# rezasalatin/PINN_depthEstimation

Measured on AMD Instinct MI355X. Metric: collocation-point residuals/sec (fwd+PDE-grad+Adam), higher is better.
Workload: dtype f32; 1 GPU; BASELINE configs[1]: 3->8x64 tanh->4 MLP, Navier_Stokes residual, 1048576 synthetic (t,x,y) points per GPU, full-batch Adam step; points_per_gpu=1048576, global_points=1048576, params=29636, parallelism=dp1, engine=0, allreduce_bytes=0

## Files before the change

pinn_depthestimation_amd/csrc/fused_kernel.h:

```cpp
#pragma once
#include <string.h>
#include <type_traits>
#include "common.h"
#include "residuals.h"

namespace pinn {

typedef float f4 __attribute__((ext_vector_type(4)));

constexpr int FUSED_WAVES = 4;
constexpr int FUSED_W16_WAVES = 3;
constexpr int FUSED_FLUSH_ROWS = 4;
constexpr int FUSED_THREADS = FUSED_WAVES * 64;
constexpr int TB_FLOATS = 256;
constexpr int TB_PER_WAVE = 8;
constexpr int MAX_SUMS = 12;
constexpr int MSE_SUM0 = 4;

struct FusedParams {
  int d_in, d_out, L, act;
  int dir_col[PINN_MAX_DIRS];
  int64_t N, n_tiles;
  const float* X;
  const float* Wp;
  const float* WTp;
  const float* Bp;
  float* scratch;
  int64_t scratch_per_wave;
  float* Y; float* dY;
  int loss_kind;
  int residual_id;
  int out_col[PINN_MAX_ROLES];
  int q_of[PINN_MAX_DIRS];
  float thr, anchor; int xcol;
  const float* scale;
  int n_cols;
  int mse_col[PINN_MAX_ROLES];
  const float* T;
  int64_t n_split;
  const float* mse_scale;
  float* wg_sums;
  float* wg_grads;
  int acc_lds;
  int PW, PB;
  int lds_acc_floats;
  int batch_T;
  int io1;
  uint32_t drop_seed, drop_thresh;
  float drop_scale, drop_keep;
  const float* gY;
  const float* gdY;
};

__device__ __forceinline__ f4 mfma4(float a, float b, f4 c) {
  return __builtin_amdgcn_mfma_f32_16x16x4f32(a, b, c, 0, 0, 0);
}

template <int WP> __device__ __forceinline__ int w_off_p(int l) { return l == 0 ? 0 : WP * 16 + (l - 1) * WP * WP; }
template <int WP> __device__ __forceinline__ int b_off_p(int l) { return l * WP; }

template <int NT_IN, int NT_OUT>
__device__ __forceinline__ void load_w(const float* __restrict__ Wl, f4 (&w)[NT_OUT][NT_IN], int m, int kq) {
  constexpr int LDW = 16 * NT_IN;
#pragma unroll
  for (int MT = 0; MT < NT_OUT; ++MT)
#pragma unroll
    for (int kt = 0; kt < NT_IN; ++kt)
      w[MT][kt] = *reinterpret_cast<const f4*>(Wl + (16 * MT + m) * LDW + 16 * kt + 4 * kq);
}

template <int NT_IN, int NT_OUT, int K1, int KR = 4>
__device__ __forceinline__ void gemm_chain(const f4 (&w)[NT_OUT][NT_IN], const f4 (&bin)[K1][NT_IN],
                                           f4 (&acc)[K1][NT_OUT]) {
#pragma unroll
  for (int MT = 0; MT < NT_OUT; ++MT)
#pragma unroll
    for (int kt = 0; kt < NT_IN; ++kt)
#pragma unroll
      for (int r = 0; r < KR; ++r)
#pragma unroll
        for (int c = 0; c < K1; ++c) acc[c][MT] = mfma4(w[MT][kt][r], bin[c][kt][r], acc[c][MT]);
}


template <int NT_IN>
__device__ __forceinline__ void load_wblk(const float* __restrict__ Wl, int MT, f4 (&w)[NT_IN], int m, int kq) {
#pragma unroll
  for (int kt = 0; kt < NT_IN; ++kt)
    w[kt] = *reinterpret_cast<const f4*>(Wl + (16 * MT + m) * (16 * NT_IN) + 16 * kt + 4 * kq);
}

struct NoMid { __device__ __forceinline__ void operator()() const {} };
template <int NT_IN, int NT_OUT, int K1, class Mid = NoMid>
__device__ __forceinline__ void gemm_stream(const float* __restrict__ Wl, const float* __restrict__ Wnext,
                                            f4 (&wa)[NT_IN], const f4 (&bin)[K1][NT_IN], f4 (&acc)[K1][NT_OUT],
                                            int m, int kq, const Mid& mid = Mid()) {
  constexpr int MID_BLOCK = NT_OUT >= 3 ? 1 : 0;
#pragma unroll
  for (int MT = 0; MT < NT_OUT; ++MT) {
    f4 wb[NT_IN];
    if (MT + 1 < NT_OUT) load_wblk<NT_IN>(Wl, MT + 1, wb, m, kq);
    else load_wblk<NT_IN>(Wnext, 0, wb, m, kq);
    if (MT == MID_BLOCK) mid();
#pragma unroll
    for (int kt = 0; kt < NT_IN; ++kt)
#pragma unroll
      for (int r = 0; r < 4; ++r)
#pragma unroll
        for (int c = 0; c < K1; ++c) acc[c][MT] = mfma4(wa[kt][r], bin[c][kt][r], acc[c][MT]);
    __builtin_amdgcn_sched_barrier(0);
#pragma unroll
    for (int kt = 0; kt < NT_IN; ++kt) wa[kt] = wb[kt];
  }
}

template <int NT, int K1>
__device__ __forceinline__ void zero_tiles(f4 (&v)[K1][NT]) {
#pragma unroll
  for (int c = 0; c < K1; ++c)
#pragma unroll
    for (int MT = 0; MT < NT; ++MT) v[c][MT] = f4{0.f, 0.f, 0.f, 0.f};
}

template <int NT, int K1>
__device__ __forceinline__ void init_bias(const float* __restrict__ b, f4 (&acc)[K1][NT], int q) {
#pragma unroll
  for (int MT = 0; MT < NT; ++MT) {
    acc[0][MT] = *reinterpret_cast<const f4*>(b + 16 * MT + 4 * q);
#pragma unroll
    for (int c = 1; c < K1; ++c) acc[c][MT] = f4{0.f, 0.f, 0.f, 0.f};
  }
}

template <int ACT, int NT, int K1>
__device__ __forceinline__ void activate(f4 (&acc)[K1][NT]) {
#pragma unroll
  for (int MT = 0; MT < NT; ++MT)
#pragma unroll
    for (int r = 0; r < 4; ++r) {
      const float z = acc[0][MT][r];
      float a, s;
      if constexpr (ACT == PINN_ACT_TANH) { a = tanh_f32(z); s = fmaf(-a, a, 1.f); }
      else { a = z > 0.f ? z : 0.01f * z; s = z > 0.f ? 1.f : 0.01f; }
      acc[0][MT][r] = a;
#pragma unroll
      for (int c = 1; c < K1; ++c) acc[c][MT][r] *= s;
    }
}

template <int ACT, int NT, int K1>
__device__ __forceinline__ void activate_adjoint(f4 (&G)[K1][NT], const f4 (&A)[K1][NT]) {
#pragma unroll
  for (int MT = 0; MT < NT; ++MT)
#pragma unroll
    for (int r = 0; r < 4; ++r) {
      const float a = A[0][MT][r];
      if constexpr (ACT == PINN_ACT_TANH) {
        const float s = fmaf(-a, a, 1.f);
        float cross = 0.f;
#pragma unroll
        for (int c = 1; c < K1; ++c) {
          cross = fmaf(G[c][MT][r], A[c][MT][r], cross);
          G[c][MT][r] *= s;
        }
        G[0][MT][r] = fmaf(-2.f * a, cross, s * G[0][MT][r]);
      } else {
        const float s = a > 0.f ? 1.f : 0.01f;
#pragma unroll
        for (int c = 0; c < K1; ++c) G[c][MT][r] *= s;
      }
    }
}


struct DropLane {
  uint32_t h0, hi, thresh;
  float scale, keep_p;
  __device__ __forceinline__ void init(uint32_t seed, uint32_t thr, float sc, float kp, int64_t point) {
    h0 = dropout_fmix(seed ^ ((uint32_t)point * 0x9E3779B1u));
    hi = (uint32_t)((uint64_t)point >> 32);
    thresh = thr; scale = sc; keep_p = kp;
  }
  __device__ __forceinline__ float mask(int layer, int unit) const {
    const uint32_t x = h0 ^ (((uint32_t)layer * 0x01000193u + (uint32_t)unit) * 0x9E3779B1u + hi);
    return dropout_fmix(x) >= thresh ? scale : 0.f;
  }
};

template <int NT>
__device__ __forceinline__ void load_bias(const float* __restrict__ b, f4 (&bias)[NT], int q) {
#pragma unroll
  for (int MT = 0; MT < NT; ++MT) bias[MT] = *reinterpret_cast<const f4*>(b + 16 * MT + 4 * q);
}
template <int ACT, int NT, int K1, bool DROP = false>
__device__ __forceinline__ void activate_to(const f4 (&acc)[K1][NT], const f4 (&bias)[NT], f4 (&a)[K1][NT],
                                            const DropLane* dl = nullptr, int layer = 0, int q = 0) {
#pragma unroll
  for (int MT = 0; MT < NT; ++MT)
#pragma unroll
    for (int r = 0; r < 4; ++r) {
      const float z = acc[0][MT][r] + bias[MT][r];
      float av, s;
      if constexpr (ACT == PINN_ACT_TANH) { av = tanh_f32(z); s = fmaf(-av, av, 1.f); }
      else { av = z > 0.f ? z : 0.01f * z; s = z > 0.f ? 1.f : 0.01f; }
      if constexpr (DROP) {
        const float m = dl->mask(layer, 16 * MT + 4 * q + r);
        av *= m; s *= m;
      }
      a[0][MT][r] = av;
#pragma unroll
      for (int c = 1; c < K1; ++c) a[c][MT][r] = acc[c][MT][r] * s;
    }
}
template <int ACT, int NT, int K1, bool DROP = false>
__device__ __forceinline__ void activate_adjoint_to(const f4 (&G)[K1][NT], const f4 (&A)[K1][NT], f4 (&Z)[K1][NT],
                                                    const DropLane* dl = nullptr, int layer = 0, int q = 0) {
#pragma unroll
  for (int MT = 0; MT < NT; ++MT)
#pragma unroll
    for (int r = 0; r < 4; ++r) {
      float a = A[0][MT][r];
      if constexpr (DROP) a *= dl->keep_p;
      if constexpr (ACT == PINN_ACT_TANH) {
        float s = fmaf(-a, a, 1.f);
        if constexpr (DROP) s *= dl->mask(layer, 16 * MT + 4 * q + r);
        float cross = 0.f;
#pragma unroll
        for (int c = 1; c < K1; ++c) {
          cross = fmaf(G[c][MT][r], A[c][MT][r], cross);
          Z[c][MT][r] = G[c][MT][r] * s;
        }
        Z[0][MT][r] = fmaf(-2.f * a, cross, s * G[0][MT][r]);
      } else {
        const float s = a > 0.f ? 1.f : 0.01f;
#pragma unroll
        for (int c = 0; c < K1; ++c) Z[c][MT][r] = G[c][MT][r] * s;
      }
    }
}

template <int NT, int K1>
__device__ __forceinline__ void spill(float* __restrict__ slot, const f4 (&v)[K1][NT], int lane) {
#pragma unroll
  for (int c = 0; c < K1; ++c)
#pragma unroll
    for (int MT = 0; MT < NT; ++MT) *reinterpret_cast<f4*>(slot + (c * NT + MT) * 256 + lane * 4) = v[c][MT];
}
template <int NT, int K1>
__device__ __forceinline__ void unspill(const float* __restrict__ slot, f4 (&v)[K1][NT], int lane) {
#pragma unroll
  for (int c = 0; c < K1; ++c)
#pragma unroll
    for (int MT = 0; MT < NT; ++MT) v[c][MT] = *reinterpret_cast<const f4*>(slot + (c * NT + MT) * 256 + lane * 4);
}

__device__ __forceinline__ void transpose_write(float* __restrict__ tb, f4 v, int p, int q) {
  *reinterpret_cast<f4*>(tb + p * 16 + 4 * (q ^ (p & 3))) = v;
}
template <bool CONSECUTIVE = false>
__device__ __forceinline__ f4 transpose_read(const float* __restrict__ tb, int p, int q) {
  f4 o;
#pragma unroll
  for (int s = 0; s < 4; ++s) {
    const int pt = CONSECUTIVE ? 4 * q + s : 4 * s + q;
    o[s] = tb[pt * 16 + 4 * ((p >> 2) ^ (pt & 3)) + (p & 3)];
  }
  return o;
}

__device__ __forceinline__ void transpose_write2(float* __restrict__ tb, f4 v, int p, int q) {
  float* d = tb + (4 * q) * 16 + 4 * (((p >> 2) + 2 * q) & 3) + (p & 3);
#pragma unroll
  for (int r = 0; r < 4; ++r) d[r * 16] = v[r];
}
__device__ __forceinline__ f4 transpose_read2(const float* __restrict__ tb, int p, int q) {
  return *reinterpret_cast<const f4*>(tb + p * 16 + 4 * ((q + 2 * (p >> 2)) & 3));
}

constexpr int MAX_LOCKS = 128;

template <bool LDSACC>
struct GradSink {
  static constexpr bool LDS = LDSACC;
  float* acc;
  int* locks;
  __device__ __forceinline__ void lock(int l, int lane) const {
    if (lane == 0) {
      int expected = 0;
      while (!__hip_atomic_compare_exchange_strong(locks + l, &expected, 1, __ATOMIC_ACQUIRE, __ATOMIC_RELAXED,
                                                   __HIP_MEMORY_SCOPE_WORKGROUP)) {
        expected = 0;
        __builtin_amdgcn_s_sleep(1);
      }
    }
    __builtin_amdgcn_fence(__ATOMIC_ACQUIRE, "workgroup");
    __builtin_amdgcn_wave_barrier();
  }
  __device__ __forceinline__ void unlock(int l, int lane) const {
    __builtin_amdgcn_wave_barrier();
    __builtin_amdgcn_fence(__ATOMIC_RELEASE, "workgroup");
    if (lane == 0) __hip_atomic_store(locks + l, 0, __ATOMIC_RELEASE, __HIP_MEMORY_SCOPE_WORKGROUP);
  }
  __device__ __forceinline__ void add1(int idx, float v) const { acc[idx] += v; }
};

template <int MT_N, int NT_N, int K1, class Sink>
__device__ __forceinline__ void weight_grad(const Sink& sink, int layer, int woff, int boff, const f4 (&Z)[K1][MT_N],
                                            const f4 (&A)[K1][NT_N], float* __restrict__ tb, int lane) {
  const int p = lane & 15, q = lane >> 4;
  f4 dw[MT_N][NT_N];
  float bs[MT_N];
#pragma unroll
  for (int MT = 0; MT < MT_N; ++MT)
#pragma unroll
    for (int NT = 0; NT < NT_N; ++NT) dw[MT][NT] = f4{0.f, 0.f, 0.f, 0.f};
  f4 early[Sink::LDS ? 1 : MT_N][Sink::LDS ? 1 : NT_N];
  if constexpr (!Sink::LDS) {
    sink.lock(layer, lane);
#pragma unroll
    for (int MT = 0; MT < MT_N; ++MT)
#pragma unroll
      for (int NT = 0; NT < NT_N; ++NT)
        early[MT][NT] = *reinterpret_cast<const f4*>(sink.acc + woff + ((MT * NT_N + NT) * 64 + lane) * 4);
  }
  f4 zt[2][MT_N], at[2][NT_N];
  auto stage = [&](int c, f4 (&z)[MT_N], f4 (&a)[NT_N]) {
#pragma unroll
    for (int MT = 0; MT < MT_N; ++MT) transpose_write2(tb + MT * TB_FLOATS, Z[c][MT], p, q);
#pragma unroll
    for (int NT = 0; NT < NT_N; ++NT) transpose_write2(tb + (4 + NT) * TB_FLOATS, A[c][NT], p, q);
#pragma unroll
    for (int MT = 0; MT < MT_N; ++MT) z[MT] = transpose_read2(tb + MT * TB_FLOATS, p, q);
#pragma unroll
    for (int NT = 0; NT < NT_N; ++NT) a[NT] = transpose_read2(tb + (4 + NT) * TB_FLOATS, p, q);
  };
  stage(0, zt[0], at[0]);
#pragma unroll
  for (int c = 0; c < K1; ++c) {
    __builtin_amdgcn_sched_barrier(0);
    if (c + 1 < K1) stage(c + 1, zt[(c + 1) & 1], at[(c + 1) & 1]);
    __builtin_amdgcn_sched_barrier(0);
    if (c == 0) {
#pragma unroll
      for (int MT = 0; MT < MT_N; ++MT) bs[MT] = (zt[0][MT][0] + zt[0][MT][1]) + (zt[0][MT][2] + zt[0][MT][3]);
    }
#pragma unroll
    for (int s = 0; s < 4; ++s)
#pragma unroll
      for (int MT = 0; MT < MT_N; ++MT)
#pragma unroll
        for (int NT = 0; NT < NT_N; ++NT) dw[MT][NT] = mfma4(zt[c & 1][MT][s], at[c & 1][NT][s], dw[MT][NT]);
  }
#pragma unroll
  for (int MT = 0; MT < MT_N; ++MT) {
    float t = bs[MT];
    t += __shfl_xor(t, 16, 64);
    t += __shfl_xor(t, 32, 64);
    bs[MT] = t;
  }
  if constexpr (!Sink::LDS) {
#pragma unroll
    for (int MT = 0; MT < MT_N; ++MT)
#pragma unroll
      for (int NT = 0; NT < NT_N; ++NT)
        *reinterpret_cast<f4*>(sink.acc + woff + ((MT * NT_N + NT) * 64 + lane) * 4) = early[MT][NT] + dw[MT][NT];
  } else {
    sink.lock(layer, lane);
    constexpr int FR = FUSED_FLUSH_ROWS < MT_N ? FUSED_FLUSH_ROWS : MT_N;
#pragma unroll
    for (int M0 = 0; M0 < MT_N; M0 += FR) {
      f4 cur[FR][NT_N];
#pragma unroll
      for (int MT = M0; MT < M0 + FR && MT < MT_N; ++MT)
#pragma unroll
        for (int NT = 0; NT < NT_N; ++NT)
          cur[MT - M0][NT] = *reinterpret_cast<const f4*>(sink.acc + woff + ((MT * NT_N + NT) * 64 + lane) * 4);
      __builtin_amdgcn_sched_barrier(0);
      __builtin_amdgcn_sched_barrier(0);
#pragma unroll
      for (int MT = M0; MT < M0 + FR && MT < MT_N; ++MT)
#pragma unroll
        for (int NT = 0; NT < NT_N; ++NT)
          *reinterpret_cast<f4*>(sink.acc + woff + ((MT * NT_N + NT) * 64 + lane) * 4) = cur[MT - M0][NT] + dw[MT][NT];
    }
  }
  if (q == 0) {
#pragma unroll
    for (int MT = 0; MT < MT_N; ++MT) sink.add1(boff + 16 * MT + p, bs[MT]);
  }
  sink.unlock(layer, lane);
}

__device__ __forceinline__ float pick4(f4 v, int i) {
  return i == 0 ? v[0] : (i == 1 ? v[1] : (i == 2 ? v[2] : v[3]));
}
__device__ __forceinline__ float gather_out(f4 tile, int o, int p) {
  return __shfl(pick4(tile, o & 3), p + 16 * (o >> 2), 64);
}
template <int K1>
__device__ __forceinline__ f4 pick_q(const f4 (&out)[K1][1], int qi) {
  f4 v = out[0][0];
#pragma unroll
  for (int c = 1; c < K1; ++c) v = (qi == c) ? out[c][0] : v;
  return v;
}

template <int K1>
struct ScatterMap {
  int role_of[4];
  int cinv[K1];
};

template <int K1, int NC, int NR, bool ACCUM = false>
__device__ __forceinline__ void scatter_adjoint(float* __restrict__ tb, const float (&g)[NC][NR],
                                                const ScatterMap<K1>& sm, f4 (&G)[K1][1], bool valid, int p, int q) {
  if (q == 0) {
#pragma unroll
    for (int c = 0; c < NC; ++c)
#pragma unroll
      for (int r = 0; r < NR; ++r) tb[(c * NR + r) * 16 + p] = g[c][r];
  }
  __builtin_amdgcn_wave_barrier();
#pragma unroll
  for (int ce = 0; ce < K1; ++ce)
#pragma unroll
    for (int r2 = 0; r2 < 4; ++r2) {
      const int ci = sm.cinv[ce], ro = sm.role_of[r2];
      const bool ok = valid && ci >= 0 && ci < NC && ro >= 0;
      const float val = tb[ok ? (ci * NR + ro) * 16 + p : p];
      G[ce][0][r2] = (ACCUM ? G[ce][0][r2] : 0.f) + (ok ? val : 0.f);
    }
  __builtin_amdgcn_wave_barrier();
}

template <class RES, int K1, bool GRAD>
__device__ __forceinline__ void residual_tile(const FusedParams& P, const f4 (&out)[K1][1], f4 (&G)[K1][1],
                                              float (&sums)[MAX_SUMS], const ScatterMap<K1>& sm,
                                              float* __restrict__ tb, bool valid, bool masked, int p, int q,
                                              bool primary = true) {
  constexpr int NR = RES::NR, ND = RES::ND, NT = RES::NT;
  float v[1 + ND][NR], g[1 + ND][NR], sq[NT], sc[NT];
#pragma unroll
  for (int c = 0; c <= ND; ++c) {
    const f4 tile = (c == 0) ? out[0][0] : pick_q<K1>(out, P.q_of[c - 1]);
#pragma unroll
    for (int r = 0; r < NR; ++r) v[c][r] = gather_out(tile, P.out_col[r], p);
  }
#pragma unroll
  for (int t = 0; t < NT; ++t) sc[t] = GRAD ? P.scale[t] : 0.f;
  if constexpr (std::is_same<RES, ResContinuity>::value)
    RES::template eval<GRAD>(v, sc, g, sq, P.residual_id == PINN_RES_CONTINUITY_ONLY, masked, P.anchor);
  else
    RES::template eval<GRAD>(v, sc, g, sq);
  if (valid && q == 0 && primary) {
#pragma unroll
    for (int t = 0; t < NT; ++t) sums[t] += sq[t];
  }
  if constexpr (GRAD) scatter_adjoint<K1, 1 + ND, NR>(tb, g, sm, G, valid, p, q);
}

template <int K1>
__device__ __forceinline__ void build_scatter_maps(const FusedParams& P, int q, ScatterMap<K1>& sm, ScatterMap<K1>& sm_mse) {
#pragma unroll
  for (int r2 = 0; r2 < 4; ++r2) {
    int ro = -1, rm = -1;
    for (int r = PINN_MAX_ROLES - 1; r >= 0; --r) {
      ro = (P.out_col[r] == 4 * q + r2) ? r : ro;
      rm = (r < P.n_cols && P.mse_col[r] == 4 * q + r2) ? r : rm;
    }
    sm.role_of[r2] = ro;
    sm_mse.role_of[r2] = rm;
  }
  sm.cinv[0] = 0; sm_mse.cinv[0] = 0;
#pragma unroll
  for (int ce = 1; ce < K1; ++ce) {
    int ci = -1;
    for (int d = PINN_MAX_DIRS - 1; d >= 0; --d) ci = (P.q_of[d] == ce) ? 1 + d : ci;
    sm.cinv[ce] = ci;
    sm_mse.cinv[ce] = -1;
  }
}

constexpr int EPI_GENERIC = 0, EPI_NS = 1, EPI_PE = 2, EPI_CONT = 3, EPI_ADJ = 4, EPI_FIELD = 5;

template <int K1>
__device__ __forceinline__ void load_adjoint(const FusedParams& P, f4 (&G)[K1][1], int64_t pt, bool valid, int q) {
#pragma unroll
  for (int r = 0; r < 4; ++r) {
    const int o = 4 * q + r;
    const bool ok = valid && o < P.d_out;
    G[0][0][r] = (ok && P.gY != nullptr) ? P.gY[pt * P.d_out + o] : 0.f;
#pragma unroll
    for (int c = 1; c < K1; ++c)
      G[c][0][r] = (ok && P.gdY != nullptr) ? P.gdY[((int64_t)(c - 1) * P.N + pt) * P.d_out + o] : 0.f;
  }
}

template <class RES, int K1>
__device__ __forceinline__ void field_tile(const FusedParams& P, const f4 (&out)[K1][1], int64_t pt, bool valid,
                                           bool masked, int p, int q) {
  constexpr int NR = RES::NR, ND = RES::ND, NF = RES::NF;
  float v[1 + ND][NR], f[NF];
#pragma unroll
  for (int c = 0; c <= ND; ++c) {
    const f4 tile = (c == 0) ? out[0][0] : pick_q<K1>(out, P.q_of[c - 1]);
#pragma unroll
    for (int r = 0; r < NR; ++r) v[c][r] = gather_out(tile, P.out_col[r], p);
  }
  if constexpr (std::is_same<RES, ResContinuity>::value)
    RES::fields(v, f, P.residual_id == PINN_RES_CONTINUITY_ONLY, masked, P.anchor);
  else
    RES::fields(v, f);
  if (valid && q == 0) {
#pragma unroll
    for (int t = 0; t < NF; ++t) P.Y[(int64_t)t * P.N + pt] = f[t];
  }
}
template <int K1>
__device__ __forceinline__ void field_epilogue(const FusedParams& P, const f4 (&out)[K1][1], int64_t pt, int64_t ptc,
                                               bool valid, int p, int q) {
  static_assert(K1 == 3 || K1 == 4, "EPI_FIELD: K1 = 1 + the residual's directions");
  if constexpr (K1 == 4) field_tile<ResNavierStokes, K1>(P, out, pt, valid, false, p, q);
  else if (P.residual_id == PINN_RES_PHYSICS_EQUATION) field_tile<ResPhysicsEquation, K1>(P, out, pt, valid, false, p, q);
  else {
    const bool masked = P.residual_id == PINN_RES_CONTINUITY_ONLY && P.X[ptc * P.d_in + P.xcol] < P.thr;
    field_tile<ResContinuity, K1>(P, out, pt, valid, masked, p, q);
  }
}

template <int K1, bool GRAD, bool SPLIT, int EPI = EPI_GENERIC>
__device__ __forceinline__ void loss_epilogue_impl(const FusedParams& P, const f4 (&out)[K1][1], f4 (&G)[K1][1],
                                              float (&sums)[MAX_SUMS], const ScatterMap<K1>& sm,
                                              const ScatterMap<K1>& sm_mse, float* __restrict__ tb, int64_t pt,
                                              int64_t ptc, bool valid, int p, int q, bool primary = true) {
  static_assert(EPI != EPI_ADJ, "EPI_ADJ has no epilogue: k_fused calls load_adjoint instead");
  static_assert(EPI != EPI_FIELD, "EPI_FIELD has its own epilogue: k_fused calls field_epilogue instead");
  if constexpr (EPI != EPI_GENERIC) {
#pragma unroll
    for (int c = 0; c < K1; ++c) G[c][0] = f4{0.f, 0.f, 0.f, 0.f};
    if constexpr (EPI == EPI_NS) {
      if constexpr (K1 >= 4) residual_tile<ResNavierStokes, K1, GRAD>(P, out, G, sums, sm, tb, valid, false, p, q, primary);
    } else if constexpr (EPI == EPI_PE) {
      if constexpr (K1 >= 3) residual_tile<ResPhysicsEquation, K1, GRAD>(P, out, G, sums, sm, tb, valid, false, p, q, primary);
    } else {
      if constexpr (K1 >= 3) {
        const bool masked = P.residual_id == PINN_RES_CONTINUITY_ONLY && P.X[ptc * P.d_in + P.xcol] < P.thr;
        residual_tile<ResContinuity, K1, GRAD>(P, out, G, sums, sm, tb, valid, masked, p, q, primary);
      }
    }
    return;
  }
  if (P.Y != nullptr && valid && primary) {
#pragma unroll
    for (int r = 0; r < 4; ++r) {
      const int o = 4 * q + r;
      if (o < P.d_out) {
        P.Y[pt * P.d_out + o] = out[0][0][r];
        if (P.dY != nullptr) {
#pragma unroll
          for (int c = 1; c < K1; ++c) P.dY[((int64_t)(c - 1) * P.N + pt) * P.d_out + o] = out[c][0][r];
        }
      }
    }
  }
#pragma unroll
  for (int c = 0; c < K1; ++c) G[c][0] = f4{0.f, 0.f, 0.f, 0.f};
  const bool valid_r = SPLIT ? (valid && pt < P.n_split) : valid;
  const bool valid_m = SPLIT ? (valid && pt >= P.n_split) : valid;
  if (P.loss_kind & 1) {
    if (P.residual_id == PINN_RES_NAVIER_STOKES) {
      if constexpr (K1 >= 4) residual_tile<ResNavierStokes, K1, GRAD>(P, out, G, sums, sm, tb, valid_r, false, p, q, primary);
    } else if (P.residual_id == PINN_RES_PHYSICS_EQUATION) {
      if constexpr (K1 >= 3) residual_tile<ResPhysicsEquation, K1, GRAD>(P, out, G, sums, sm, tb, valid_r, false, p, q, primary);
    } else {
      if constexpr (K1 >= 3) {
        const bool masked = P.residual_id == PINN_RES_CONTINUITY_ONLY && P.X[ptc * P.d_in + P.xcol] < P.thr;
        residual_tile<ResContinuity, K1, GRAD>(P, out, G, sums, sm, tb, valid_r, masked, p, q, primary);
      }
    }
  }
  if (P.loss_kind & 2) {
    float gm[1][PINN_MAX_ROLES];
#pragma unroll
    for (int j = 0; j < PINN_MAX_ROLES; ++j) {
      gm[0][j] = 0.f;
      if (j < P.n_cols) {
        const float y = gather_out(out[0][0], P.mse_col[j], p);
        const int64_t trow = SPLIT ? (valid_m ? ptc - P.n_split : 0) : ptc;
        const float d = P.T[trow * P.n_cols + j] - y;
        if (valid_m && q == 0 && primary) sums[MSE_SUM0 + j] += d * d;
        if (GRAD) gm[0][j] = -2.f * P.mse_scale[j] * d;
      }
    }
    if constexpr (GRAD) scatter_adjoint<K1, 1, PINN_MAX_ROLES, true>(tb, gm, sm_mse, G, valid_m, p, q);
  }
}

template <int K1, bool GRAD, bool SPLIT_OK = true, int EPI = EPI_GENERIC>
__device__ __forceinline__ void loss_epilogue(const FusedParams& P, const f4 (&out)[K1][1], f4 (&G)[K1][1],
                                              float (&sums)[MAX_SUMS], const ScatterMap<K1>& sm,
                                              const ScatterMap<K1>& sm_mse, float* __restrict__ tb, int64_t pt,
                                              int64_t ptc, bool valid, int p, int q, bool primary = true) {
  if constexpr (SPLIT_OK && EPI == EPI_GENERIC) {
    if (P.n_split >= 0) {
      loss_epilogue_impl<K1, GRAD, true>(P, out, G, sums, sm, sm_mse, tb, pt, ptc, valid, p, q, primary);
      return;
    }
  }
  loss_epilogue_impl<K1, GRAD, false, EPI>(P, out, G, sums, sm, sm_mse, tb, pt, ptc, valid, p, q, primary);
}

#ifdef PINN_DIAG
#define PINN_STAMP(i)                                                                      \
  do {                                                                                     \
    unsigned long long t_;                                                                 \
    __builtin_amdgcn_sched_barrier(0);                                                     \
    asm volatile("s_waitcnt vmcnt(0) lgkmcnt(0)\n\ts_memtime %0\n\ts_waitcnt lgkmcnt(0)" : "=s"(t_)::"memory"); \
    __builtin_amdgcn_sched_barrier(0);                                                     \
    diag[i] += t_ - tprev;                                                                 \
    tprev = t_;                                                                            \
  } while (0)
#else
#define PINN_STAMP(i) do { } while (0)
#endif

template <int WP, int K1, bool GRAD, bool LDSACC, int ACT, int EPI = EPI_GENERIC, int KRO = 0, bool DROP = false>
__global__ __launch_bounds__(FUSED_THREADS, WP == 16 ? FUSED_W16_WAVES : FUSED_WAVES / 4) void k_fused(const FusedParams P) {
  static_assert(!DROP || (ACT == PINN_ACT_TANH && KRO == 0), "dropout instances: tanh, natural unit order");
  static_assert(EPI != EPI_ADJ || (GRAD && KRO == 0 && !DROP), "external-adjoint instances: gradient pass, natural unit order, no dropout");
  static_assert(EPI != EPI_FIELD || (!GRAD && !LDSACC && KRO == 0 && !DROP), "field instances: forward only, natural unit order, no dropout");
  constexpr bool IO1 = KRO > 0;
  constexpr int KRI = IO1 ? 1 : 4;
  constexpr int KRL = IO1 ? KRO : 4;
  extern __shared__ __attribute__((aligned(16))) float smem[];
  constexpr int NTH = WP / 16;
  const int lane = threadIdx.x & 63, wave = threadIdx.x >> 6;
  const int p = lane & 15, q = lane >> 4;
  float* lacc = smem;
  int* locks = reinterpret_cast<int*>(smem + P.lds_acc_floats);
  float* tb = smem + P.lds_acc_floats + MAX_LOCKS + wave * (TB_PER_WAVE * TB_FLOATS);
  float* lsum = smem + P.lds_acc_floats + MAX_LOCKS + FUSED_WAVES * TB_PER_WAVE * TB_FLOATS;
  const int PP = P.PW + P.PB;
  GradSink<LDSACC> sink;
  sink.acc = LDSACC ? lacc : P.wg_grads + (int64_t)blockIdx.x * PP;
  sink.locks = locks;
  if (GRAD) {
    if (LDSACC) {
      for (int i = threadIdx.x; i < PP; i += FUSED_THREADS) lacc[i] = 0.f;
    }
    if (threadIdx.x < MAX_LOCKS) locks[threadIdx.x] = 0;
    __syncthreads();
  }
  float sums[MAX_SUMS];
#pragma unroll
  for (int j = 0; j < MAX_SUMS; ++j) sums[j] = 0.f;

  ScatterMap<K1> sm, sm_mse;
  build_scatter_maps<K1>(P, q, sm, sm_mse);
  const int nw = gridDim.x * FUSED_WAVES;
  const int gw = EPI == EPI_ADJ ? wave * (int)gridDim.x + (int)blockIdx.x : (int)blockIdx.x * FUSED_WAVES + wave;
  float* __restrict__ scr = P.scratch + (int64_t)gw * P.scratch_per_wave;
  const float* __restrict__ Wp_ = P.Wp;
  const float* __restrict__ WTp_ = P.WTp;
  const float* __restrict__ Bp_ = P.Bp;
  constexpr int SLOT = K1 * NTH * 256;
  const int L = P.L;

#ifdef PINN_DIAG
  unsigned long long diag[12] = {0, 0, 0, 0, 0, 0, 0, 0, 0, 0, 0, 0}, tprev = __builtin_amdgcn_s_memtime();
#endif
  auto load_x = [&](int64_t t, f4& x) {
    int64_t pc = t * 16 + p;
    pc = pc < P.N ? pc : P.N - 1;
#pragma unroll
    for (int r = 0; r < 4; ++r) {
      const int f = IO1 ? (r == 0 ? q : 16) : 4 * q + r;
      x[r] = (f < P.d_in) ? P.X[pc * P.d_in + f] : 0.f;
    }
  };
  f4 xnext;
  load_x(gw < P.n_tiles ? gw : 0, xnext);
  for (int64_t tile = gw; tile < P.n_tiles; tile += nw) {
    PINN_STAMP(11);
    const int64_t pt = tile * 16 + p;
    const bool valid = pt < P.N;
    const int64_t ptc = valid ? pt : P.N - 1;
    DropLane dl;
    if constexpr (DROP) dl.init(P.drop_seed, P.drop_thresh, P.drop_scale, P.drop_keep, pt);
    const f4 xcur = xnext;
    load_x(tile + nw < P.n_tiles ? tile + nw : tile, xnext);
    auto input_jet = [&](f4 (&b)[K1][1]) {
#pragma unroll
      for (int r = 0; r < 4; ++r) {
        const int f = 4 * q + r;
        b[0][0][r] = xcur[r];
#pragma unroll
        for (int c = 1; c < K1; ++c) b[c][0][r] = (f == P.dir_col[c - 1]) ? 1.f : 0.f;
      }
    };
    f4 b0[K1][1];
    input_jet(b0);
    f4 a[K1][NTH];
    f4 ws[NTH];
    {
      f4 w0[NTH][1];
      load_w<1, NTH>(Wp_, w0, p, q);
      load_wblk<NTH>(Wp_ + w_off_p<WP>(L > 1 ? 1 : L), 0, ws, p, q);
      f4 bias[NTH];
      load_bias<NTH>(Bp_ + b_off_p<WP>(0), bias, q);
      f4 acc0[K1][NTH];
      zero_tiles<NTH, K1>(acc0);
      gemm_chain<1, NTH, K1, KRI>(w0, b0, acc0);
      PINN_STAMP(0);
      activate_to<ACT, NTH, K1, DROP>(acc0, bias, a, &dl, 0, q);
    }
    PINN_STAMP(1);
    for (int l = 1; l < L; ++l) {
      f4 bias[NTH];
      load_bias<NTH>(Bp_ + b_off_p<WP>(l), bias, q);
      f4 nx[K1][NTH];
      zero_tiles<NTH, K1>(nx);
      auto sp = [&]() { if (GRAD) spill<NTH, K1>(scr + (l - 1) * SLOT, a, lane); };
      gemm_stream<NTH, NTH, K1>(Wp_ + w_off_p<WP>(l), Wp_ + w_off_p<WP>(l + 1), ws, a, nx, p, q, sp);
      PINN_STAMP(0);
      activate_to<ACT, NTH, K1, DROP>(nx, bias, a, &dl, l, q);
      PINN_STAMP(1);
    }
    f4 G[K1][1];
    f4 out[K1][1];
    if constexpr (EPI == EPI_ADJ) {
      load_adjoint<K1>(P, G, pt, valid, q);
      load_wblk<NTH>(WTp_ + w_off_p<WP>(L > 1 ? L - 1 : 0), 0, ws, p, q);
    } else {
      f4 bias_o[1];
      load_bias<1>(Bp_ + b_off_p<WP>(L), bias_o, q);
      zero_tiles<1, K1>(out);
      gemm_stream<NTH, 1, K1>(Wp_ + w_off_p<WP>(L), WTp_ + w_off_p<WP>(L > 1 ? L - 1 : 0), ws, a, out, p, q);
      out[0][0] += bias_o[0];
    }
    f4 wtl[NTH][1];
    f4 ai[K1][NTH];
    if constexpr (GRAD) load_w<1, NTH>(WTp_ + w_off_p<WP>(L), wtl, p, q);

    if constexpr (EPI == EPI_FIELD) field_epilogue<K1>(P, out, pt, ptc, valid, p, q);
    else if constexpr (EPI != EPI_ADJ) loss_epilogue<K1, GRAD, (WP < 64), EPI>(P, out, G, sums, sm, sm_mse, tb, pt, ptc, valid, p, q);

    PINN_STAMP(2);
    if constexpr (GRAD) {
      weight_grad<1, NTH, K1>(sink, L, w_off_p<WP>(L), P.PW + b_off_p<WP>(L), G, a, tb, lane);
      f4 z[K1][NTH];
      {
        f4 g[K1][NTH];
        zero_tiles<NTH, K1>(g);
        gemm_chain<1, NTH, K1, KRL>(wtl, G, g);
        activate_adjoint_to<ACT, NTH, K1, DROP>(g, a, z, &dl, L - 1, q);
      }
      for (int l = L - 1; l >= 1; --l) {
        PINN_STAMP(3);
        f4 g2[K1][NTH];
        zero_tiles<NTH, K1>(g2);
        auto ld = [&]() { unspill<NTH, K1>(scr + (l - 1) * SLOT, ai, lane); };
        gemm_stream<NTH, NTH, K1>(WTp_ + w_off_p<WP>(l), WTp_ + w_off_p<WP>(l >= 2 ? l - 1 : 1), ws, z, g2, p, q, ld);
        PINN_STAMP(6);
        weight_grad<NTH, NTH, K1>(sink, l, w_off_p<WP>(l), P.PW + b_off_p<WP>(l), z, ai, tb, lane);
        PINN_STAMP(5);
        activate_adjoint_to<ACT, NTH, K1, DROP>(g2, ai, z, &dl, l - 1, q);
        PINN_STAMP(4);
      }
      {
        f4 b1[K1][1];
        input_jet(b1);
        weight_grad<NTH, 1, K1>(sink, 0, 0, P.PW + b_off_p<WP>(0), z, b1, tb, lane);
      }
    }
    PINN_STAMP(7);
  }
#ifdef PINN_DIAG
  if (blockIdx.x == 0 && threadIdx.x == 0 && GRAD) {
    unsigned long long tot = 0;
    for (int i = 0; i < 12; ++i) tot += diag[i];
    printf("DIAG cycles/wave: fwd_gemm %llu fwd_act+spill %llu out+residual %llu | unspill_wait %llu adjoint %llu wgrad(transp+mfma+flush) %llu bwd_gemm %llu first/last-layer %llu loop-top %llu | total %llu\n",
           diag[0], diag[1], diag[2], diag[3], diag[4], diag[5], diag[6], diag[7], diag[11], tot);
  }
#endif

  if constexpr (EPI == EPI_FIELD) return;
#pragma unroll
  for (int j = 0; j < MAX_SUMS; ++j) {
    float v = sums[j];
#pragma unroll
    for (int off = 32; off > 0; off >>= 1) v += __shfl_down(v, off, 64);
    if (lane == 0) lsum[wave * MAX_SUMS + j] = v;
  }
  __syncthreads();
  if (threadIdx.x < MAX_SUMS) {
    float v = 0.f;
#pragma unroll
    for (int w = 0; w < FUSED_WAVES; ++w) v += lsum[w * MAX_SUMS + threadIdx.x];
    P.wg_sums[(int64_t)blockIdx.x * MAX_SUMS + threadIdx.x] = v;
  }
  if (GRAD && LDSACC) {
    float* dst = P.wg_grads + (int64_t)blockIdx.x * PP;
    for (int i = threadIdx.x; i < PP; i += FUSED_THREADS) dst[i] = lacc[i];
  }
}

template <int WP>
int launch_fused(int K1, bool grad, const FusedParams& P, int grid, size_t lds_bytes, hipStream_t s);
template <int WP>
int launch_fused_adj(int K1, const FusedParams& P, int grid, size_t lds_bytes, hipStream_t s);
template <int WP>
int launch_fused_field(int K1, const FusedParams& P, int grid, size_t lds_bytes, hipStream_t s);

}
```

pinn_depthestimation_amd/csrc/residuals.h:

```cpp
#pragma once
#include <hip/hip_runtime.h>

namespace pinn {

struct ResNavierStokes {
  static constexpr int NR = 4, ND = 3, NT = 3;
  template <bool GRAD>
  __device__ static inline void eval(const float (&v)[1 + ND][NR], const float* scale,
                                     float (&g)[1 + ND][NR], float (&sq)[NT]) {
    const float h = v[0][0], z = v[0][1], u = v[0][2], w = v[0][3];
    const float z_t = v[1][1], u_t = v[1][2], w_t = v[1][3];
    const float h_x = v[2][0], z_x = v[2][1], u_x = v[2][2], w_x = v[2][3];
    const float h_y = v[3][0], z_y = v[3][1], u_y = v[3][2], w_y = v[3][3];
    const float G = 9.81f;
    const float CB = (float)(3.0 / 16.0 * 9.81 * (0.78 * 0.78));
    const float H = h + z;
    const float Hx = h_x + z_x, Hy = h_y + z_y;
    const float hu_x = Hx * u + H * u_x;
    const float hv_y = Hy * w + H * w_y;
    const float Fbr_x = CB * Hx * H, Fbr_y = CB * Hy * H;
    const float fc = z_t + hu_x + hv_y;
    const float fmx = u_t + u * u_x + w * u_y + G * z_x + Fbr_x;
    const float fmy = w_t + u * w_x + w * w_y + G * z_y + Fbr_y;
    sq[0] = fc * fc; sq[1] = fmx * fmx; sq[2] = fmy * fmy;
    if (GRAD) {
      const float rc = 2.f * scale[0] * fc, rx = 2.f * scale[1] * fmx, ry = 2.f * scale[2] * fmy;
      const float gh = rc * (u_x + w_y) + CB * (rx * Hx + ry * Hy);
      g[0][0] = gh; g[0][1] = gh;
      g[0][2] = rc * Hx + rx * u_x + ry * w_x;
      g[0][3] = rc * Hy + rx * u_y + ry * w_y;
      g[1][0] = 0.f; g[1][1] = rc; g[1][2] = rx; g[1][3] = ry;
      const float ghx = rc * u + rx * CB * H;
      g[2][0] = ghx; g[2][1] = ghx + rx * G;
      g[2][2] = rc * H + rx * u; g[2][3] = ry * u;
      const float ghy = rc * w + ry * CB * H;
      g[3][0] = ghy; g[3][1] = ghy + ry * G;
      g[3][2] = rx * w; g[3][3] = rc * H + ry * w;
    }
  }
  static constexpr int NF = 3;
  __device__ static inline void fields(const float (&v)[1 + ND][NR], float (&f)[NF]) {
    const float h = v[0][0], z = v[0][1], u = v[0][2], w = v[0][3];
    const float z_t = v[1][1], u_t = v[1][2], w_t = v[1][3];
    const float h_x = v[2][0], z_x = v[2][1], u_x = v[2][2], w_x = v[2][3];
    const float h_y = v[3][0], z_y = v[3][1], u_y = v[3][2], w_y = v[3][3];
    const float G = 9.81f;
    const float CB = (float)(3.0 / 16.0 * 9.81 * (0.78 * 0.78));
    const float H = h + z;
    const float Hx = h_x + z_x, Hy = h_y + z_y;
    const float hu_x = Hx * u + H * u_x;
    const float hv_y = Hy * w + H * w_y;
    const float Fbr_x = CB * Hx * H, Fbr_y = CB * Hy * H;
    f[0] = z_t + hu_x + hv_y;
    f[1] = u_t + u * u_x + w * u_y + G * z_x + Fbr_x;
    f[2] = w_t + u * w_x + w * w_y + G * z_y + Fbr_y;
  }
};

struct ResPhysicsEquation {
  static constexpr int NR = 6, ND = 2, NT = 3;
  template <bool GRAD>
  __device__ static inline void eval(const float (&v)[1 + ND][NR], const float* scale,
                                     float (&g)[1 + ND][NR], float (&sq)[NT]) {
    const float h = v[0][0], U = v[0][1], V = v[0][2], eta = v[0][3];
    const float U_x = v[1][1], V_x = v[1][2], e_x = v[1][3];
    const float U_y = v[2][1], V_y = v[2][2], e_y = v[2][3];
    const float G = 9.81f, RHO = 1025.f;
    const float RC = (float)(1025 * 0.002);
    const float tbx = (RC * U) * fabsf(U);
    const float tby = (RC * V) * fabsf(V);
    const float D = 1.0f / (RHO * (eta + h));
    const float fc = U_x + V_y;
    const float fx = U * U_x + V * U_y + G * e_x + D * tbx;
    const float fy = U * V_x + V * V_y + G * e_y + D * tby;
    sq[0] = fc * fc; sq[1] = fx * fx; sq[2] = fy * fy;
    if (GRAD) {
      const float rc = 2.f * scale[0] * fc, rx = 2.f * scale[1] * fx, ry = 2.f * scale[2] * fy;
#pragma unroll
      for (int c = 0; c < 1 + ND; ++c)
#pragma unroll
        for (int r = 0; r < NR; ++r) g[c][r] = 0.f;
      const float dD = -RHO * D * D;
      const float gS = dD * (rx * tbx + ry * tby);
      g[0][0] = gS; g[0][3] = gS;
      g[0][1] = rx * (U_x + D * RC * 2.f * fabsf(U)) + ry * V_x;
      g[0][2] = rx * U_y + ry * (V_y + D * RC * 2.f * fabsf(V));
      g[1][1] = rc + rx * U;
      g[1][2] = ry * U;
      g[1][3] = rx * G;
      g[2][1] = rx * V;
      g[2][2] = rc + ry * V;
      g[2][3] = ry * G;
    }
  }
  static constexpr int NF = 3;
  __device__ static inline void fields(const float (&v)[1 + ND][NR], float (&f)[NF]) {
    const float h = v[0][0], U = v[0][1], V = v[0][2], eta = v[0][3];
    const float U_x = v[1][1], V_x = v[1][2], e_x = v[1][3];
    const float U_y = v[2][1], V_y = v[2][2], e_y = v[2][3];
    const float G = 9.81f, RHO = 1025.f;
    const float RC = (float)(1025 * 0.002);
    const float tbx = (RC * U) * fabsf(U);
    const float tby = (RC * V) * fabsf(V);
    const float D = 1.0f / (RHO * (eta + h));
    f[0] = U_x + V_y;
    f[1] = U * U_x + V * U_y + G * e_x + D * tbx;
    f[2] = U * V_x + V * V_y + G * e_y + D * tby;
  }
};

struct ResContinuity {
  static constexpr int NR = 3, ND = 2, NT = 3;
  template <bool GRAD>
  __device__ static inline void eval(const float (&v)[1 + ND][NR], const float* scale,
                                     float (&g)[1 + ND][NR], float (&sq)[NT],
                                     bool anchor_on, bool masked, float anchor) {
    const float h = v[0][0], U = v[0][1], V = v[0][2];
    const float h_x = v[1][0], U_x = v[1][1];
    const float h_y = v[2][0], V_y = v[2][2];
    const float fc = h_x * U + h * U_x + h_y * V + h * V_y;
    sq[0] = fc * fc;
    const float da = (anchor_on && masked) ? (h - anchor) : 0.f;
    sq[1] = da * da;
    sq[2] = (anchor_on && masked) ? 1.f : 0.f;
    if (GRAD) {
      const float rc = 2.f * scale[0] * fc;
#pragma unroll
      for (int c = 0; c < 1 + ND; ++c)
#pragma unroll
        for (int r = 0; r < NR; ++r) g[c][r] = 0.f;
      g[0][0] = rc * (U_x + V_y) + (anchor_on ? 2.f * scale[1] * da : 0.f);
      g[0][1] = rc * h_x;
      g[0][2] = rc * h_y;
      g[1][0] = rc * U; g[1][1] = rc * h;
      g[2][0] = rc * V; g[2][2] = rc * h;
    }
  }
  static constexpr int NF = 2;
  __device__ static inline void fields(const float (&v)[1 + ND][NR], float (&f)[NF],
                                       bool anchor_on, bool masked, float anchor) {
    const float h = v[0][0], U = v[0][1], V = v[0][2];
    const float h_x = v[1][0], U_x = v[1][1];
    const float h_y = v[2][0], V_y = v[2][2];
    f[0] = h_x * U + h * U_x + h_y * V + h * V_y;
    f[1] = (anchor_on && masked) ? (h - anchor) : 0.f;
  }
};

__device__ inline float tanh_f32(float x) {
  const float ax = fabsf(x);
  const float x2 = x * x;
  float p = -5.70498872745e-3f;
  p = fmaf(p, x2, 2.06390887954e-2f);
  p = fmaf(p, x2, -5.37397155531e-2f);
  p = fmaf(p, x2, 1.33314422036e-1f);
  p = fmaf(p, x2, -3.33332819422e-1f);
  const float small = fmaf(p * x2, x, x);
  const float e = __expf(2.f * ax);
  const float big = copysignf(fmaf(-2.f, __builtin_amdgcn_rcpf(e + 1.f), 1.f), x);
  return ax < 0.625f ? small : big;
}

}
```

Before: 167.5 million residual-points/s.

## Pack tanh into float2 ops, skip unit-tangent staging, use permlane reductions

Rewrites the tanh activation path to work on float2 vectors so the compiler can emit packed FMA/mul instructions. In the layer-0 weight gradient, the input tangent directions are one-hot, so it builds them in registers instead of staging them through LDS transposes. The bias-sum reductions switch from shfl_xor to permlane16/32 swaps, and the LDS bias accumulator load is hoisted into the flush loop. This trades code complexity and the assumption that input tangents are unit vectors selected by dir_col for fewer VALU and LDS operations.

```diff
diff --git a/pinn_depthestimation_amd/csrc/fused_kernel.h b/pinn_depthestimation_amd/csrc/fused_kernel.h
--- a/pinn_depthestimation_amd/csrc/fused_kernel.h
+++ b/pinn_depthestimation_amd/csrc/fused_kernel.h
@@ -195,6 +195,23 @@
 template <int ACT, int NT, int K1, bool DROP = false>
 __device__ __forceinline__ void activate_to(const f4 (&acc)[K1][NT], const f4 (&bias)[NT], f4 (&a)[K1][NT],
                                             const DropLane* dl = nullptr, int layer = 0, int q = 0) {
+  if constexpr (ACT == PINN_ACT_TANH && !DROP) {
+#pragma unroll
+    for (int MT = 0; MT < NT; ++MT)
+#pragma unroll
+      for (int h = 0; h < 4; h += 2) {
+        const f2 z = f2{acc[0][MT][h], acc[0][MT][h + 1]} + f2{bias[MT][h], bias[MT][h + 1]};
+        const f2 av = tanh_f32x2(z);
+        const f2 s = __builtin_elementwise_fma(-av, av, f2{1.f, 1.f});
+        a[0][MT][h] = av[0]; a[0][MT][h + 1] = av[1];
+#pragma unroll
+        for (int c = 1; c < K1; ++c) {
+          const f2 t = f2{acc[c][MT][h], acc[c][MT][h + 1]} * s;
+          a[c][MT][h] = t[0]; a[c][MT][h + 1] = t[1];
+        }
+      }
+    return;
+  }
 #pragma unroll
   for (int MT = 0; MT < NT; ++MT)
 #pragma unroll
@@ -275,6 +292,15 @@
 }
 __device__ __forceinline__ f4 transpose_read2(const float* __restrict__ tb, int p, int q) {
   return *reinterpret_cast<const f4*>(tb + p * 16 + 4 * ((q + 2 * (p >> 2)) & 3));
+}
+
+__device__ __forceinline__ float add_xor16(float t) {
+  const auto r = __builtin_amdgcn_permlane16_swap(__float_as_uint(t), __float_as_uint(t), false, false);
+  return __uint_as_float(r[0]) + __uint_as_float(r[1]);
+}
+__device__ __forceinline__ float add_xor32(float t) {
+  const auto r = __builtin_amdgcn_permlane32_swap(__float_as_uint(t), __float_as_uint(t), false, false);
+  return __uint_as_float(r[0]) + __uint_as_float(r[1]);
 }
 
 constexpr int MAX_LOCKS = 128;
@@ -304,12 +330,14 @@
   __device__ __forceinline__ void add1(int idx, float v) const { acc[idx] += v; }
 };
 
-template <int MT_N, int NT_N, int K1, class Sink>
+template <int MT_N, int NT_N, int K1, bool UNIT_A = false, class Sink>
 __device__ __forceinline__ void weight_grad(const Sink& sink, int layer, int woff, int boff, const f4 (&Z)[K1][MT_N],
-                                            const f4 (&A)[K1][NT_N], float* __restrict__ tb, int lane) {
+                                            const f4 (&A)[K1][NT_N], float* __restrict__ tb, int lane,
+                                            const int* __restrict__ dir_col = nullptr) {
+  static_assert(!UNIT_A || NT_N == 1, "unit tangents: the layer-0 input block");
   const int p = lane & 15, q = lane >> 4;
   f4 dw[MT_N][NT_N];
-  float bs[MT_N];
+  float bs[MT_N], bcur[MT_N];
 #pragma unroll
   for (int MT = 0; MT < MT_N; ++MT)
 #pragma unroll
@@ -327,12 +355,20 @@
   auto stage = [&](int c, f4 (&z)[MT_N], f4 (&a)[NT_N]) {
 #pragma unroll
     for (int MT = 0; MT < MT_N; ++MT) transpose_write2(tb + MT * TB_FLOATS, Z[c][MT], p, q);
-#pragma unroll
-    for (int NT = 0; NT < NT_N; ++NT) transpose_write2(tb + (4 + NT) * TB_FLOATS, A[c][NT], p, q);
+    const bool unit = UNIT_A && c > 0;
+    if (!unit) {
+#pragma unroll
+      for (int NT = 0; NT < NT_N; ++NT) transpose_write2(tb + (4 + NT) * TB_FLOATS, A[c][NT], p, q);
+    }
 #pragma unroll
     for (int MT = 0; MT < MT_N; ++MT) z[MT] = transpose_read2(tb + MT * TB_FLOATS, p, q);
-#pragma unroll
-    for (int NT = 0; NT < NT_N; ++NT) a[NT] = transpose_read2(tb + (4 + NT) * TB_FLOATS, p, q);
+    if (!unit) {
+#pragma unroll
+      for (int NT = 0; NT < NT_N; ++NT) a[NT] = transpose_read2(tb + (4 + NT) * TB_FLOATS, p, q);
+    } else {
+      const float e = (p == dir_col[c - 1]) ? 1.f : 0.f;
+      a[0] = f4{e, e, e, e};
+    }
   };
   stage(0, zt[0], at[0]);
 #pragma unroll
@@ -353,10 +389,7 @@
   }
 #pragma unroll
   for (int MT = 0; MT < MT_N; ++MT) {
-    float t = bs[MT];
-    t += __shfl_xor(t, 16, 64);
-    t += __shfl_xor(t, 32, 64);
-    bs[MT] = t;
+    bs[MT] = add_xor32(add_xor16(bs[MT]));
   }
   if constexpr (!Sink::LDS) {
 #pragma unroll
@@ -375,6 +408,10 @@
 #pragma unroll
         for (int NT = 0; NT < NT_N; ++NT)
           cur[MT - M0][NT] = *reinterpret_cast<const f4*>(sink.acc + woff + ((MT * NT_N + NT) * 64 + lane) * 4);
+      if (M0 == 0) {
+#pragma unroll
+        for (int MT = 0; MT < MT_N; ++MT) bcur[MT] = sink.acc[boff + 16 * MT + p];
+      }
       __builtin_amdgcn_sched_barrier(0);
       __builtin_amdgcn_sched_barrier(0);
 #pragma unroll
@@ -386,7 +423,10 @@
   }
   if (q == 0) {
 #pragma unroll
-    for (int MT = 0; MT < MT_N; ++MT) sink.add1(boff + 16 * MT + p, bs[MT]);
+    for (int MT = 0; MT < MT_N; ++MT) {
+      if constexpr (Sink::LDS) sink.acc[boff + 16 * MT + p] = bcur[MT] + bs[MT];
+      else sink.add1(boff + 16 * MT + p, bs[MT]);
+    }
   }
   sink.unlock(layer, lane);
 }
@@ -397,11 +437,12 @@
 __device__ __forceinline__ float gather_out(f4 tile, int o, int p) {
   return __shfl(pick4(tile, o & 3), p + 16 * (o >> 2), 64);
 }
+__device__ __forceinline__ f4 select4(bool take, f4 a, f4 b) { return take ? a : b; }
 template <int K1>
 __device__ __forceinline__ f4 pick_q(const f4 (&out)[K1][1], int qi) {
   f4 v = out[0][0];
 #pragma unroll
-  for (int c = 1; c < K1; ++c) v = (qi == c) ? out[c][0] : v;
+  for (int c = 1; c < K1; ++c) v = select4(qi == c, out[c][0], v);
   return v;
 }
 
@@ -770,7 +811,7 @@
       {
         f4 b1[K1][1];
         input_jet(b1);
-        weight_grad<NTH, 1, K1>(sink, 0, 0, P.PW + b_off_p<WP>(0), z, b1, tb, lane);
+        weight_grad<NTH, 1, K1, LDSACC>(sink, 0, 0, P.PW + b_off_p<WP>(0), z, b1, tb, lane, P.dir_col);
       }
     }
     PINN_STAMP(7);
diff --git a/pinn_depthestimation_amd/csrc/residuals.h b/pinn_depthestimation_amd/csrc/residuals.h
--- a/pinn_depthestimation_amd/csrc/residuals.h
+++ b/pinn_depthestimation_amd/csrc/residuals.h
@@ -161,4 +161,22 @@
   return ax < 0.625f ? small : big;
 }
 
+typedef float f2 __attribute__((ext_vector_type(2)));
+__device__ inline f2 tanh_f32x2(f2 x) {
+  const f2 x2 = x * x;
+  f2 p = f2{-5.70498872745e-3f, -5.70498872745e-3f};
+  p = __builtin_elementwise_fma(p, x2, f2{2.06390887954e-2f, 2.06390887954e-2f});
+  p = __builtin_elementwise_fma(p, x2, f2{-5.37397155531e-2f, -5.37397155531e-2f});
+  p = __builtin_elementwise_fma(p, x2, f2{1.33314422036e-1f, 1.33314422036e-1f});
+  p = __builtin_elementwise_fma(p, x2, f2{-3.33332819422e-1f, -3.33332819422e-1f});
+  const f2 small = __builtin_elementwise_fma(p * x2, x, x);
+  const f2 t = (x + x) * f2{0x1.715476p+0f, 0x1.715476p+0f};
+  const f2 e = f2{__builtin_amdgcn_exp2f(fabsf(t[0])), __builtin_amdgcn_exp2f(fabsf(t[1]))};
+  const f2 d = e + f2{1.f, 1.f};
+  const f2 r = f2{__builtin_amdgcn_rcpf(d[0]), __builtin_amdgcn_rcpf(d[1])};
+  const f2 big = __builtin_elementwise_fma(f2{-2.f, -2.f}, r, f2{1.f, 1.f});
+  return f2{fabsf(x[0]) < 0.625f ? small[0] : copysignf(big[0], x[0]),
+            fabsf(x[1]) < 0.625f ? small[1] : copysignf(big[1], x[1])};
 }
+
+}
```

Measured after the change: 169.7 million residual-points/s, median of 6. +1.4%, better.
